# UCL-SML/Doubly-Stochastic-DGP

Hardware: AMD Instinct MI355X
Metric: ELBO-steps/sec (higher is better)
Workload: dtype f64

## Files before the change

doubly-stochastic-dgp_amd/csrc/model_kernels.hpp:

```cpp
#pragma once
__device__ __forceinline__ double softplus_d(double x) { return x > 0 ? x + log1p(exp(-x)) : log1p(exp(x)); }
__device__ __forceinline__ double sigmoid_d(double x) { return 1.0 / (1.0 + exp(-x)); }
__device__ __forceinline__ double kvar_of(const LayerDev& v, const double* __restrict__ theta) {
  const double rv = theta[v.off_kvar];
  return v.kvar_identity ? rv : softplus_d(rv) + SOFTPLUS_LOWER;
}

template <bool WAVE_TILES>
__device__ void prep_body(const LayerDev& v, const double* __restrict__ theta, double* __restrict__ lik_const, int64_t off_lik,
                          int lik_gauss, int bx, int nprep) {
  const int tid0 = bx * blockDim.x + threadIdx.x, nth = nprep * blockDim.x;
  if (tid0 == 0) {
    const double rv = theta[v.off_kvar];
    const double var = kvar_of(v, theta);
    double wv = 0.0, dwv = 0.0;
    if (v.has_white) {
      const double rw = theta[v.off_wvar];
      wv = softplus_d(rw) + SOFTPLUS_LOWER;
      dwv = sigmoid_d(rw);
    }
    v.hyp[HYP_VAR] = var; v.hyp[HYP_WVAR] = wv; v.hyp[HYP_KDIAG] = var + wv;
    v.hyp[HYP_DVAR] = v.kvar_identity ? 1.0 : sigmoid_d(rv); v.hyp[HYP_DWVAR] = dwv;
    if (blockIdx.y == 0 && lik_gauss) {
      const double rl = theta[off_lik];
// ... 968 lines not shown
      }
      s = sum_wave(s);
      if (lane == 0) gl_s[q] = -2.0 * ils[q] * ils[q] * ils[q] * s + v.hyp_red[2 + q];
    }
    __syncthreads();
    if (threadIdx.x < Din) {
      const double gl = gl_s[threadIdx.x];
      if (v.ard)
        grad[v.off_kls + threadIdx.x] = gl * v.hyp[HYP_ILS + Din + threadIdx.x];
      else
        iso = gl;
    }
  } else {
    for (int q = threadIdx.x; q < Din; q += 256) {
      double s = 0.0;
      for (int b0 = 0; b0 < parts; b0 += 8) {
        double x[8];
#pragma unroll
        for (int u = 0; u < 8; ++u) x[u] = v.hyp2part[(b0 + u < parts ? b0 + u : parts - 1) * stride + 2 + q];
#pragma unroll
        for (int u = 0; u < 8; ++u)
          if (b0 + u < parts) s += x[u];
      }
      const double gl = -2.0 * ils[q] * ils[q] * ils[q] * s + v.hyp_red[2 + q];
      if (v.ard)
        grad[v.off_kls + q] = gl * v.hyp[HYP_ILS + Din + q];
      else
        iso += gl;
    }
  }
  iso = block_sum_256(iso, sh);
  if (!v.ard && threadIdx.x == 0) grad[v.off_kls] = iso * v.hyp[HYP_ILS + Din];
}
__device__ __forceinline__ void adam_sweep(double* __restrict__ theta, const double* __restrict__ grad, double* __restrict__ m,
                                           double* __restrict__ v, const double* __restrict__ mask, int64_t n, double lr_t, double b1,
                                           double b2, double eps, double want, int64_t first, int64_t nthreads) {
  typedef double d2 __attribute__((ext_vector_type(2)));
  const int64_t npair = n >> 1;
  for (int64_t k0 = first; k0 < npair; k0 += 4 * nthreads) {
    d2 mk[4];
    bool act[4];
#pragma unroll
    for (int u = 0; u < 4; ++u) {
      const int64_t k = k0 + u * nthreads;
      mk[u] = *reinterpret_cast<const d2*>(mask + 2 * (k < npair ? k : first));
    }
#pragma unroll
    for (int u = 0; u < 4; ++u) {
      const int64_t k = k0 + u * nthreads;
      act[u] = k < npair && (want == 0.0 ? (mk[u][0] != 0.0 || mk[u][1] != 0.0) : (mk[u][0] == want || mk[u][1] == want));
    }
    d2 g[4], mm[4], vv[4], th[4];
#pragma unroll
    for (int u = 0; u < 4; ++u) {
      const int64_t k = k0 + u * nthreads;
      if (act[u]) {
        g[u] = *reinterpret_cast<const d2*>(grad + 2 * k);
        mm[u] = *reinterpret_cast<const d2*>(m + 2 * k);
        vv[u] = *reinterpret_cast<const d2*>(v + 2 * k);
        th[u] = *reinterpret_cast<const d2*>(theta + 2 * k);
      }
    }
#pragma unroll
    for (int u = 0; u < 4; ++u) {
      if (!act[u]) continue;
      const int64_t k = k0 + u * nthreads;
      bool on[2];
#pragma unroll
      for (int e = 0; e < 2; ++e) {
        on[e] = want == 0.0 ? mk[u][e] != 0.0 : mk[u][e] == want;
        if (on[e]) {
          const double mi = b1 * mm[u][e] + (1.0 - b1) * g[u][e];
          const double vi = b2 * vv[u][e] + (1.0 - b2) * g[u][e] * g[u][e];
          mm[u][e] = mi;
          vv[u][e] = vi;
          th[u][e] -= lr_t * mi / (sqrt(vi) + eps);
        }
      }
      if (on[0] && on[1]) {
        *reinterpret_cast<d2*>(m + 2 * k) = mm[u];
        *reinterpret_cast<d2*>(v + 2 * k) = vv[u];
        *reinterpret_cast<d2*>(theta + 2 * k) = th[u];
      } else {
#pragma unroll
        for (int e = 0; e < 2; ++e)
          if (on[e]) {
            m[2 * k + e] = mm[u][e];
            v[2 * k + e] = vv[u][e];
            theta[2 * k + e] = th[u][e];
          }
      }
    }
  }
  if ((n & 1) && first == 0) {
    const int64_t i = n - 1;
    const bool on = want == 0.0 ? mask[i] != 0.0 : mask[i] == want;
    if (on) {
      const double gi = grad[i];
      const double mi = b1 * m[i] + (1.0 - b1) * gi;
      const double vi = b2 * v[i] + (1.0 - b2) * gi * gi;
      m[i] = mi;
      v[i] = vi;
      theta[i] -= lr_t * mi / (sqrt(vi) + eps);
    }
  }
}
__device__ __forceinline__ bool chol_failed(const LayerDev* __restrict__ layers, int L) {
  bool bad = false;
  for (int l = 0; l < L; ++l) bad |= layers[l].scal[1] != 0.0;
  return bad;
}
__global__ void k_adam(double* __restrict__ theta, const double* __restrict__ grad, double* __restrict__ m,
                       double* __restrict__ v, const double* __restrict__ mask, int64_t n, double lr_t, double b1,
                       double b2, double eps, const LayerDev* __restrict__ layers, int L) {
  if (chol_failed(layers, L)) return;
  adam_sweep(theta, grad, m, v, mask, n, lr_t, b1, b2, eps, 0.0, (int64_t)blockIdx.x * blockDim.x + threadIdx.x,
             (int64_t)gridDim.x * blockDim.x);
}

__global__ __launch_bounds__(256) void k_asm_rows(const LayerDev* __restrict__ layers, double* __restrict__ grad, double kl_w, int mp_max, int pre_on) {
  extern __shared__ __attribute__((aligned(16))) double asm_dyn[];
  __shared__ double sh[4];
  const LayerDev v = layers[blockIdx.y];
  const int tid = threadIdx.x, lane = tid & 63, wave = tid >> 6;
  const int i = (int)blockIdx.x;
  const int Mp = v.Mp, M = v.M, Din = v.D_in, Dout = v.D_out;
  if (i >= M) return;
  lptr wm = (lptr)asm_dyn;
  const int64_t MM = (int64_t)Mp * Mp;
  const double kvar = v.hyp[HYP_VAR];
  const bool pre = pre_on && (M <= 128) && (Din <= 8) && (Dout * M <= 1024);
  double pz[2][2] = {{0, 0}, {0, 0}}, pzi[2] = {0, 0}, ptz[2] = {0, 0}, ptz1 = 0.0, pq_t = 0.0, pq_n = 0.0;
  double p4p[4] = {0, 0, 0, 0}, p4u[4] = {0, 0, 0, 0}, p4t[4] = {0, 0, 0, 0};
  if (pre) {
    gcptr Zp = (gcptr)v.Zp, thinz = (gcptr)v.thinz, thinq = (gcptr)v.thinq, n4 = (gcptr)v.n4, PT = (gcptr)v.PT, U = (gcptr)v.U, Tp = (gcptr)v.Tp;
#pragma unroll
    for (int u = 0; u < 2; ++u) {
      const int q = wave + 4 * u, qc = q < Din ? q : Din - 1;
      pzi[u] = Zp[i * Din + qc];
      ptz[u] = thinz[i * v.DinP16 + qc];
#pragma unroll
      for (int w = 0; w < 2; ++w) {
        const int j = lane + 64 * w;
        pz[u][w] = Zp[(j < M ? j : M - 1) * Din + qc];
      }
    }
    ptz1 = thinz[i * v.DinP16 + Din];
    const int dq = tid < Dout ? tid : Dout - 1;
    pq_t = thinq[i * v.DP16 + dq];
    pq_n = n4[i * v.DP4 + dq];
#pragma unroll
    for (int u = 0; u < 4; ++u) {
      int e = tid + 256 * u;
      e = e < Dout * M ? e : Dout * M - 1;
      const int d = e / M, j = e - d * M;
      const int64_t p = d * MM + (int64_t)i * Mp + (j <= i ? j : i);
      p4p[u] = PT[p];
      p4u[u] = U[p];
      p4t[u] = Tp[p];
    }
  }
  double a_sum = 0.0, tr = 0.0;
  for (int j = tid; j < M; j += 256) {
    const int64_t idx = (int64_t)i * Mp + j, idt = (int64_t)j * Mp + i;
    double nn = 0.0, uu = 0.0, gsym;
    if (v.alg_g) {
      double gs = 0.0, nt = 0.0;
#pragma unroll 4
      for (int d = 0; d < Dout; ++d) {
        const double ni = v.n4[i * v.DP4 + d], nj = v.n4[j * v.DP4 + d];
        const double g1 = v.GS[d * MM + idx], g2 = v.GS[d * MM + idt], pd = v.bigred[MM + d * MM + idx];
        const double tj = v.thinq[j * v.DP16 + d], ti2 = v.thinq[i * v.DP16 + d];
        nn = fma(ni, nj, nn);
        uu += v.UU[d * MM + idx];
        gs += (g1 + g2) - pd;
        nt += ni * tj + nj * ti2;
      }
      gsym = gs + 0.5 * nt;
    } else {
#pragma unroll 4
      for (int d = 0; d < Dout; ++d) {
        nn = fma(v.n4[i * v.DP4 + d], v.n4[j * v.DP4 + d], nn);
        uu += v.UU[d * MM + idx];
      }
      gsym = 0.5 * (v.bigred[idx] + v.bigred[idt]);
    }
    const double kb = -gsym + kl_w * (0.5 * Dout * v.Kinv[idx] - 0.5 * uu - 0.5 * nn);
    double k, dk;
    if (v.kern_kind == DSDGP_KERN_RBF)
      kern_val_grad<DSDGP_KERN_RBF>(v.R2[idx], kvar, k, dk);
    else
      kern_val_grad<DSDGP_KERN_MATERN52>(v.R2[idx], kvar, k, dk);
    wm[j] = kb * dk;
    a_sum += kb * k / kvar;
    if (j == i) tr = kb;
  }
  a_sum = block_sum_256(a_sum, sh);
  tr = block_sum_256(tr, sh);
  double* __restrict__ hp = v.hyp2part + (int64_t)i * (Din + 2);
  if (tid == 0) {
    hp[0] = a_sum;
    hp[1] = tr;
  }
  const double* __restrict__ ils = v.hyp + HYP_ILS;
  if (pre) {
#pragma unroll
    for (int u = 0; u < 2; ++u) {
      const int q = wave + 4 * u;
      if (q >= Din) break;
      const double zi = pzi[u];
      double s1 = 0.0, s2 = 0.0;
#pragma unroll
      for (int w = 0; w < 2; ++w) {
        const int j = lane + 64 * w;
        if (j < M) {
          const double df = zi - pz[u][w], wj = wm[j];
          s1 = fma(wj, df, s1);
          s2 = fma(wj * df, df, s2);
        }
      }
      s1 = sum_wave(s1);
      s2 = sum_wave(s2);
      if (lane == 0) {
        const double il2 = ils[q] * ils[q];
        grad[v.off_Z + (int64_t)i * Din + q] = 4.0 * il2 * s1 - 2.0 * il2 * (ptz[u] - zi * ptz1);
        hp[2 + q] = s2;
      }
    }
    if (tid < Dout) grad[v.off_q_mu + (int64_t)i * Dout + tid] = pq_t + kl_w * pq_n;
#pragma unroll
    for (int u = 0; u < 4; ++u) {
      const int e = tid + 256 * u;
      if (e < Dout * M) {
        const int d = e / M, j = e - d * M;
        const double gq = 2.0 * p4p[u] + kl_w * (p4u[u] - (i == j ? 1.0 / p4t[u] : 0.0));
        grad[v.off_q_sqrt + ((int64_t)d * M + i) * M + j] = (j <= i) ? gq : 0.0;
      }
    }
  } else {
  for (int q = wave; q < Din; q += 4) {
    const double zi = v.Zp[i * Din + q];
    double s1 = 0.0, s2 = 0.0;
    for (int j = lane; j < M; j += 64) {
      const double df = zi - v.Zp[j * Din + q], w = wm[j];
      s1 = fma(w, df, s1);
      s2 = fma(w * df, df, s2);
    }
    s1 = sum_wave(s1);
    s2 = sum_wave(s2);
    if (lane == 0) {
      const double il2 = ils[q] * ils[q];
      grad[v.off_Z + (int64_t)i * Din + q] = 4.0 * il2 * s1 - 2.0 * il2 * (v.thinz[i * v.DinP16 + q] - zi * v.thinz[i * v.DinP16 + Din]);
      hp[2 + q] = s2;
    }
  }
  for (int d = tid; d < Dout; d += 256) grad[v.off_q_mu + (int64_t)i * Dout + d] = v.thinq[i * v.DP16 + d] + kl_w * v.n4[i * v.DP4 + d];
  {
    constexpr int NU = 4;
    for (int j0 = 0; j0 < M; j0 += 256 * NU) {
      double pt[NU], uu[NU], td = 0.0;
      auto request = [&](int d) {
        gcptr PT = (gcptr)(v.PT + d * MM + (int64_t)i * Mp), U = (gcptr)(v.U + d * MM + (int64_t)i * Mp);
#pragma unroll
        for (int u = 0; u < NU; ++u) {
          const int j = j0 + tid + 256 * u, jc = j <= i ? j : i;
          pt[u] = PT[jc];
          uu[u] = U[jc];
        }
        td = ((gcptr)v.Tp)[d * MM + (int64_t)i * Mp + i];
      };
      request(0);
      for (int d = 0; d < Dout; ++d) {
        double gq[NU];
        const double tinv = 1.0 / td;
#pragma unroll
        for (int u = 0; u < NU; ++u) {
          const int j = j0 + tid + 256 * u;
          gq[u] = (j <= i) ? 2.0 * pt[u] + kl_w * (uu[u] - (i == j ? tinv : 0.0)) : 0.0;
        }
        if (d + 1 < Dout) request(d + 1);
        double* gr = grad + v.off_q_sqrt + ((int64_t)d * M + i) * M;
#pragma unroll
        for (int u = 0; u < NU; ++u) {
          const int j = j0 + tid + 256 * u;
          if (j < M) gr[j] = gq[u];
        }
      }
    }
  }
  }
  if (v.meanAB) {
    if (v.off_mean_A >= 0)
      for (int64_t idx = (int64_t)i * 256 + tid; idx < (int64_t)Din * Dout; idx += (int64_t)M * 256)
        grad[v.off_mean_A + idx] = v.meanAB[(idx / Dout) * v.DP16 + idx % Dout];
    if (v.off_mean_b >= 0 && i == 0)
      for (int idx = tid; idx < Dout; idx += 256) grad[v.off_mean_b + idx] = v.meanAB[(int64_t)Din * v.DP16 + idx];
  }
}

struct AdamArgs {
  double* theta; double* m; double* v; const double* mask;
  int64_t n;
  double lr_t, b1, b2, eps;
  int32_t on;
};
__device__ __forceinline__ void adam_one(const AdamArgs& A, int64_t i, double g) {
  const double mi = A.b1 * A.m[i] + (1.0 - A.b1) * g;
  const double vi = A.b2 * A.v[i] + (1.0 - A.b2) * g * g;
  A.m[i] = mi;
  A.v[i] = vi;
  A.theta[i] -= A.lr_t * mi / (sqrt(vi) + A.eps);
}
struct FinArgs {
  const double* part; int nblocks; double w, kl_weight; const double* lik_const; int64_t off_lik; double* out; int L;
  int do_fin;
};
__global__ __launch_bounds__(256) void k_tail(const LayerDev* __restrict__ layers_all, int first, int La, double* __restrict__ grad,
                                              const FinArgs F, const AdamArgs A) {
  __shared__ double sh[4];
  const int b = (int)blockIdx.x;
  const bool adam_on = A.on && !chol_failed(layers_all, F.L);
  if (b < La) {
    const LayerDev v = layers_all[first + b];
    asm_hyp_final(v, grad);
    if (adam_on) {
      __syncthreads();
      const int Din = v.D_in;
      if (threadIdx.x == 0) {
        if (A.mask[v.off_kvar] != 0.0) adam_one(A, v.off_kvar, grad[v.off_kvar]);
        if (v.has_white && A.mask[v.off_wvar] != 0.0) adam_one(A, v.off_wvar, grad[v.off_wvar]);
        if (!v.ard && A.mask[v.off_kls] != 0.0) adam_one(A, v.off_kls, grad[v.off_kls]);
      }
      if (v.ard && (int)threadIdx.x < Din && A.mask[v.off_kls + threadIdx.x] != 0.0)
        adam_one(A, v.off_kls + threadIdx.x, grad[v.off_kls + threadIdx.x]);
    }
    return;
  }
  const int nf = F.do_fin ? 1 : 0;
  if (b == La && nf) {
    double a = 0.0, c = 0.0;
    for (int i = threadIdx.x; i < F.nblocks; i += 256) {
      a += F.part[2 * i];
      c += F.part[2 * i + 1];
    }
    a = block_sum_256(a, sh);
    c = block_sum_256(c, sh);
    const double kl = layers_kl_value(layers_all, F.L, sh);
    if (threadIdx.x == 0) {
      double info = 0.0;
      for (int l = 0; l < F.L; ++l)
        if (layers_all[l].scal[1] != 0.0 && info == 0.0) info = layers_all[l].scal[1];
      F.out[0] = F.w * a - F.kl_weight * kl;
      F.out[1] = F.w * a;
      F.out[2] = F.kl_weight * kl;
      F.out[3] = info;
      if (F.off_lik >= 0) {
        const double g = -F.w * c * F.lik_const[1];
        grad[F.off_lik] = g;
        if (adam_on && A.mask[F.off_lik] != 0.0) adam_one(A, F.off_lik, g);
      }
    }
    return;
  }
  if (!adam_on) return;
  adam_sweep(A.theta, grad, A.m, A.v, A.mask, A.n, A.lr_t, A.b1, A.b2, A.eps, 1.0, (int64_t)(b - La - nf) * 256 + threadIdx.x,
             (int64_t)(gridDim.x - La - nf) * 256);
}
```

doubly-stochastic-dgp_amd/csrc/model_layout.hpp:

```cpp
#pragma once
static void layout(dsdgp_model* m, char* base, size_t* total) {
  Bump b{base, 0};
  const dsdgp_model_desc& D = m->desc;
  m->layers_dev = b.take<LayerDev>(D.L);
  m->mask = b.take<double>(D.n_theta);
  m->lik_const = b.take<double>(8);
  m->scal4 = b.take<double>(8);
  const int64_t Rlast = (int64_t)m->s_max * m->n_max;
  m->lik_blocks_max = std::max(ceil_div((Rlast + 16) * D.layers[D.L - 1].D_out, 256) + 1,
                               4 * ceil_div(Rlast, 16) + 4);
  m->lik_part = b.take<double>((size_t)m->lik_blocks_max * 2);
  m->Xmb = b.take<double>((size_t)m->n_max * D.layers[0].D_in);
  m->Ymb = b.take<double>((size_t)m->n_max * D.layers[D.L - 1].D_out);
  m->lik_dmean = b.take<double>((size_t)Rlast * D.layers[D.L - 1].D_out);
  m->lik_dvar = b.take<double>((size_t)Rlast * D.layers[D.L - 1].D_out);
  m->potrf_items = b.take<PotrfItem>(D.L);
  m->gp_fwd = b.take<GemmProblem>(4 * D.L);
  m->gp_bwd1 = b.take<GemmProblem>(4 * D.L);
  m->gp_pt = b.take<GemmProblem>(2 * D.L);
  m->gp_bwd2 = b.take<GemmProblem>(D.L);
  m->gp_wz = b.take<GemmProblem>(D.L);
  m->gp_w1 = b.take<GemmProblem>(2 * D.L); m->gp_w2 = b.take<GemmProblem>(D.L); m->gp_w3 = b.take<GemmProblem>(D.L);
  m->rjobs_cap = 0;
  for (int l = 0; l < D.L; ++l) m->rjobs_cap += D.layers[l].D_out + 5;
  m->rjobs = b.take<RedJob>(m->rjobs_cap);
  bool uniform = D.L > 1 && pad_M(D.layers[0].M) >= big_mp(true);
  for (int l = 1; l < D.L; ++l) uniform = uniform && D.layers[l].M == D.layers[0].M;
  uniform = uniform && pad_M(D.layers[0].M) % 64 == 0;
  m->uniform_big = uniform;
  double *Kp_all = nullptr, *Linv_all = nullptr, *LinvT_all = nullptr, *scal_all = nullptr;
  if (uniform) {
    const size_t MM0 = (size_t)pad_M(D.layers[0].M) * pad_M(D.layers[0].M);
    Kp_all = b.take<double>(D.L * MM0); Linv_all = b.take<double>(D.L * MM0); LinvT_all = b.take<double>(D.L * MM0);
    scal_all = b.take<double>(D.L * 8);
  }
  for (int l = 0; l < D.L; ++l) {
    LayerState& S = m->L[l];
    const dsdgp_layer_desc& d = D.layers[l];
    S.d = d;
    LayerDev& v = S.dev;
// ... 122 lines not shown
```

doubly-stochastic-dgp_amd/csrc/model_schedule.hpp:

```cpp
#pragma once
static bool overlap_on(const dsdgp_model* m, int64_t n, int S) {
  const char* no = getenv("DSDGP_NO_OVERLAP");
  if (!m->overlap || (no && atoi(no))) return false;
  int mp_max = 0;
  for (int l = 0; l < m->desc.L; ++l) mp_max = std::max(mp_max, (int)m->L[l].dev.Mp);
  return n * S * (int64_t)mp_max >= (int64_t)m->force.overlap_min;
}

static int join_prep(dsdgp_model* m) {
  if (m->side_pending) {
    DS_HIP(hipStreamWaitEvent(m->ctx->stream, m->ev_prep_side, 0));
    m->side_pending = false;
  }
  return DSDGP_OK;
}

static int prepare_async(dsdgp_model* m, bool with_grad = false, bool side = false, const HeadRand* hr = nullptr,
                         const HeadGather* hg = nullptr) {
  dsdgp_ctx* ctx = m->ctx;
  const int L = m->desc.L;
  DS_TRY(join_prep(m));
  const bool keep_kuu = m->track_theta && m->kuu_valid;
  const bool unchanged = keep_kuu && m->q_dirty == -1 && (m->prepared_grad || !with_grad);
  int mp_max = 0;
// ... 399 lines not shown
  return DSDGP_OK;
}

static int launch_finalize(dsdgp_model* m, hipStream_t st) {
  DS_LAUNCH(k_finalize, dim3(1), dim3(256), 0, st, m->layers_dev, m->desc.L, m->lik_part, m->fin.nblocks, m->fin.w,
                     m->fin.kl_weight, m->lik_const, m->grad,
                     lik_has_param(m->desc.lik_kind) ? m->desc.off_lik_var : (int64_t)-1, m->fin.with_grad, m->fin.out);
  DS_HIP(hipGetLastError());
  m->fin.done = true;
  return DSDGP_OK;
}

static int backward_layers(dsdgp_model* m, int64_t n, int S, double kl_weight) {
  dsdgp_ctx* ctx = m->ctx;
  const int L = m->desc.L;
  DS_TRY(ensure_plan(m, n, S));
  const bool overlap = overlap_on(m, n, S);
  const int gfirst0 = m->desc.white ? 0 : m->grad_first;
  const bool tail_in_loop = (m->bucket_fn != nullptr && m->tail_ok && gfirst0 == 0 && !m->fuse_adam.on) ||
                            (overlap && m->force.pipe_tail != 0 && !m->desc.white);
  const bool kinv_only = overlap && !tail_in_loop && !m->desc.white && m->kinv_pending && m->side_pending;
  if (kinv_only) DS_HIP(hipStreamWaitEvent(ctx->stream, m->ev_kinv, 0));
  else DS_TRY(join_prep(m));
  const int gfirst = m->desc.white ? 0 : m->grad_first;
  const bool bucketed = m->bucket_fn != nullptr && m->tail_ok && gfirst == 0 && !m->fuse_adam.on;
  const bool pipelined = bucketed || (overlap && m->force.pipe_tail != 0 && !m->desc.white);
  auto layer_tail = [&](LayerState& St, hipStream_t st) -> int {
    DS_LAUNCH(k_reduce_grouped, dim3(St.red_blkn), dim3(256), m->red_lds, st, m->rjobs + St.red_off, St.red_n, St.red_blk0);
    DS_HIP(hipGetLastError());
    DS_TRY(gemm_launch(ctx, St.lq + St.lq_nf + St.lq_n1 + St.lq_n2, St.lq_np, St.lq_tp, st));
    if (bucketed) {
      const int l = (int)(&St - m->L);
      const LayerDev* lay1 = m->layers_dev + l;
      DS_LAUNCH(k_asm_rows, dim3(St.dev.M, 1), dim3(256), (size_t)m->mp_max_all * sizeof(double), st, lay1, m->grad, kl_weight,
                         m->mp_max_all, m->force.asm_pre);
      FinArgs F{};
      AdamArgs A{};
      DS_LAUNCH(k_tail, dim3(1), dim3(256), 0, st, m->layers_dev, l, 1, m->grad, F, A);
      DS_HIP(hipGetLastError());
      const int64_t lo = St.d.off_Z;
      const int64_t hi = (l + 1 < L) ? m->L[l + 1].d.off_Z
                                     : (lik_has_param(m->desc.lik_kind) ? m->desc.off_lik_var : m->desc.n_theta);
      m->bucket_fn(m->bucket_user, l, m->grad + lo, hi - lo, (void*)st);
    }
    return DSDGP_OK;
  };
  const bool q_only = m->grad_q_only && !m->desc.white;
  auto launch_wgrad = [&](LayerState& Sx, hipStream_t st) -> int {
    const int64_t ldx = Sx.ld_used;
    if (q_only && &Sx == &m->L[gfirst]) return wgrad_launch(ctx, Sx.wj, Sx.njobsA, Sx.totA, Sx.ns_big, ldx, ldx, st);
    return wgrad_launch(ctx, Sx.wj, Sx.njobs, Sx.tot_big, Sx.ns_big, ldx, ldx, st);
  };
  const bool defer_upper = overlap && !pipelined && (m->force.wg_defer == 2 || (m->force.wg_defer < 0 && L - gfirst >= 4));
  for (int l = L - 1; l >= gfirst; --l) {
    LayerState& St = m->L[l];
    const LayerDev& v = St.dev;
    const bool last = (l == L - 1);
    const int64_t Rin = St.Rin_used, ld = St.ld_used;
    const int rep = St.rep_used;
    const bool fused = (last && m->fused_last) || (!last && l >= 1);
    const bool skip_chain = q_only && l == gfirst;
    const bool in_chain = !fused && !last && !skip_chain && m->force.adj_fuse != 0 && !St.c_used && !St.gemm &&
                          sm_adj_fusable(v.Mp, ld / 16, v.D_in, v.D_out);
    if (!fused && !in_chain)
      DS_LAUNCH(k_adj_prep, dim3(ceil_div(ld, 256), std::max(v.DP16, v.DinP16)), dim3(256), 0, ctx->stream, last ? nullptr : St.dF,
                         last ? m->lik_dmean : nullptr, last ? m->lik_dvar : nullptr, St.z_used, St.zs_s, St.zs_n,
                         St.zs_d, n, St.var, St.X_used, Rin, rep, v.D_in, v.D_out, v.DP16, v.DinP16, m->desc.jitter, ld,
                         St.MB, St.VB, St.XT1, v.D_out + St.prop, St.prop);
    DS_HIP(hipGetLastError());
    const bool on_main = overlap && l == gfirst && L - gfirst > 1;
// ... 68 lines not shown
    }
    DS_HIP(hipGetLastError());
    if (m->desc.white) {
      DS_LAUNCH(k_white_lbar, dim3(32, L), dim3(256), 0, ctx->stream, m->layers_dev);
      DS_TRY(gemm_launch(ctx, m->gp_w1, 2 * L, m->t_w1));
      DS_LAUNCH(k_white_phi, dim3(32, L), dim3(256), 0, ctx->stream, m->layers_dev);
      DS_TRY(gemm_launch(ctx, m->gp_w2, L, m->t_w2));
      DS_TRY(gemm_launch(ctx, m->gp_w3, L, m->t_w3));
    } else if (gfirst > 0) {
      for (int l = gfirst; l < L; ++l) {
        LayerState& Sq = m->L[l];
        DS_TRY(gemm_launch(ctx, Sq.lq + Sq.lq_nf + Sq.lq_n1 + Sq.lq_n2, Sq.lq_np, Sq.lq_tp));
      }
    } else {
      DS_TRY(gemm_launch(ctx, m->gp_pt, m->n_pt, m->t_pt));
    }
  }
  const LayerDev* lay = m->layers_dev + gfirst;
  const int La = L - gfirst;
  if (bucketed) {
    FinArgs F{m->lik_part, m->fin.nblocks, m->fin.w, m->fin.kl_weight, m->lik_const,
              lik_has_param(m->desc.lik_kind) ? m->desc.off_lik_var : (int64_t)-1, m->fin.out, L, 1};
    AdamArgs A{};
    DS_LAUNCH(k_tail, dim3(1), dim3(256), 0, ctx->stream, m->layers_dev, 0, 0, m->grad, F, A);
    DS_HIP(hipGetLastError());
    m->fin.done = true;
    const int64_t lo = lik_has_param(m->desc.lik_kind) ? m->desc.off_lik_var : m->desc.n_theta;
    const bool tail_scalars = m->fin.out == m->grad + m->desc.n_theta;
    m->bucket_fn(m->bucket_user, L, m->grad + lo, (m->desc.n_theta - lo) + (tail_scalars ? 4 : 0), (void*)ctx->stream);
    if (!tail_scalars) m->bucket_fn(m->bucket_user, L + 1, m->fin.out, 4, (void*)ctx->stream);
    return DSDGP_OK;
  }
  if (m->tail_ok) {
    DS_LAUNCH(k_asm_rows, dim3(m->m_max_all, La), dim3(256), (size_t)m->mp_max_all * sizeof(double), ctx->stream, lay, m->grad,
                       kl_weight, m->mp_max_all, m->force.asm_pre);
    FinArgs F{m->lik_part, m->fin.nblocks, m->fin.w, m->fin.kl_weight, m->lik_const,
              lik_has_param(m->desc.lik_kind) ? m->desc.off_lik_var : (int64_t)-1, m->fin.out, L, 1};
    AdamArgs A{m->theta, m->adam_m, m->adam_v, m->mask, m->desc.n_theta, m->fuse_adam.lr_t, m->fuse_adam.b1, m->fuse_adam.b2,
               m->fuse_adam.eps, (m->fuse_adam.on && gfirst == 0) ? 1 : 0};
    const int nadam = A.on ? (int)std::min<int64_t>(2048, ceil_div(m->desc.n_theta, 512)) : 0;
    DS_LAUNCH(k_tail, dim3(La + 1 + nadam), dim3(256), 0, ctx->stream, m->layers_dev, gfirst, La, m->grad, F, A);
    DS_HIP(hipGetLastError());
    m->fin.done = true;
    return DSDGP_OK;
  }
  DS_LAUNCH(k_asm_kbar, dim3(m->kuu_blocks, La), dim3(256), 0, ctx->stream, lay, kl_weight);
  if (m->n_wz) DS_TRY(gemm_launch(ctx, m->gp_wz, m->n_wz, m->t_wz));
  if (m->need_hyp_part) DS_LAUNCH(k_asm_hyp_part, dim3(NPART, La), dim3(256), 0, ctx->stream, lay);
  DS_LAUNCH(k_asm_params, dim3(m->asm_blocks + 1, La), dim3(256), 0, ctx->stream, lay, m->grad, kl_weight);
  DS_HIP(hipGetLastError());
  return DSDGP_OK;
}

struct GatherSrc {
  const double *Xs, *Ys;
  const int64_t* idx;
};
static int elbo_impl(dsdgp_model* m, const double* X, const double* Y, int64_t n, int32_t S, const double* const* zs,
                     const int64_t* zstride, uint64_t seed, double data_scale, double kl_weight, int with_grad, double* out,
                     const GatherSrc* gs) {
  DS_CHECK_ARG(m && out && ((X && Y) || gs));
  DS_CHECK_ARG(!zs || zstride);
  DS_CHECK_ARG(!m->sample_w || S == m->sample_w_S);
  if (with_grad) {
    DS_CHECK_ARG(m->grad != nullptr);
  }
  dsdgp_ctx* ctx = m->ctx;
  const int L = m->desc.L;
  bool z_side = false, z_head = false;
  const bool ovl = overlap_on(m, n, S);
  HeadRand hr{};
  if (m->head_ok) {
// ... 146 lines not shown
```

doubly-stochastic-dgp_amd/csrc/model_types.hpp:

```cpp
#pragma once
struct LayerDev {
  int32_t M, Mp, D_in, D_out, DP4, DP16, DinP16, kern_kind, ard, has_white, white, hyp_parts;
  int32_t kl_parts, kvar_identity;
  int64_t off_Z, off_q_mu, off_q_sqrt, off_kvar, off_kls, off_wvar;
  double *Zp, *Zs, *hyp, *Tp, *TpT, *qmu, *qmu4;
  double *Kp, *Linv, *LinvT, *Kinv, *scal;
  double *V, *nL, *Sd, *klv;
  double *U, *n4, *PT, *UU, *Kbar, *wm, *wk;
  double *bigred, *thinq, *thinz, *hyp_red;
  double* meanAB;
  int64_t off_mean_A, off_mean_b;
  double *R2, *Zp1, *WZ;
  double *klpart, *hyp2part;
  double *KS, *GS;
  int32_t alg_g, need_tpt;
  double *wLbar, *wH, *wY, *wX;
  double *ngTI, *ngTinv, *ngTbar, *ngH, *ngY, *ngX, *ngSinv, *ngA, *ngLAinv, *ngLAinvT, *ngV , *ngTheta1 , *ngScal ;
};
#define NPART 32
#define PREP_BLOCKS 64
#define WIDE_DIN 32

struct RedJob {
  const double* part;
// ... 61 lines not shown
  double* lik_part;
  int lik_blocks_max;
  double *lik_dmean, *lik_dvar;
  double* scal4;
  PotrfItem* potrf_items;
  GemmProblem *gp_fwd, *gp_bwd1, *gp_bwd2, *gp_w1, *gp_w2, *gp_w3;
  GemmProblem* gp_pt;
  int n_pt = 0, t_pt = 0;
  hipEvent_t ev_fork, ev_prep_side, ev_z;
  hipEvent_t ev_kinv;
  bool kinv_pending = false;
  int32_t* gemm_order = nullptr;
  int64_t gemm_order_cap = 0, gemm_order_used = 0;
  GemmLayerWs gws{};
  bool prepared_grad = false;
  bool track_theta = false;
  bool kuu_valid = false;
  int grad_first = 0;
  bool grad_pruned = false;
  bool grad_q_only = false;
  int q_dirty = -2;
  bool side_pending = false;
  int n_fwd, n_bwd1, n_bwd2, t_fwd, t_bwd1, t_bwd2, n_w, t_w1, t_w2, t_w3;
  const double* sample_w = nullptr;
  int sample_w_S = 0;
  GemmProblem* gp_wz;
  int n_wz = 0, t_wz = 0, kuu_blocks = 32, asm_blocks = 64, prep_blocks = PREP_BLOCKS;
  bool uniform_big = false;
  BigChol big_all;
  bool need_hyp_part = false;
  bool tail_ok = false;
  struct { int on; double lr_t, b1, b2, eps; } fuse_adam = {0, 0, 0, 0, 0};
  int mp_max_all = 0, m_max_all = 0;
  dsdgp_bucket_fn bucket_fn = nullptr;
  void* bucket_user = nullptr;
  double *Xmb = nullptr, *Ymb = nullptr;
  bool head_ok = false;
  bool last_deferred = false;
  LayerFwdArgs last_fwd;
  bool fused_last = false;
  struct { int nblocks; double w, kl_weight; int with_grad; double* out; bool done; } fin;
  RedJob* rjobs;
  int rjobs_cap, n_red, red_blocks;
  size_t red_lds = 0;
  int64_t plan_n;
  int plan_S;
  bool prepared;
  hipStream_t side;
  hipEvent_t ev_bwd[DSDGP_MAX_LAYERS];
  hipEvent_t ev_side;
  bool overlap;
  struct Force { int save_c = 1, cs_min_blocks = 160, cs_min_dout = 3, cs_max_dout = 1 << 20, wg_defer = -1, alg_g = -1, bwd_split = 1, pipe_tail = 0, head = 1, tail = 1, adj_fuse = 1, ext_ev = 1, lik_fuse = 1, red_ahead = 1, white_fwd = 1, gemm_mp = 512, last_fuse = 1, last_min_blocks = 1, asm_pre = 1, overlap_min = 1 << 18, wg_red = 1, wg_group = 1; } force;
};
static void parse_force(dsdgp_model* m) {
  const char* e = getenv("DSDGP_FORCE");
  if (!e) return;
  std::string str(e);
  size_t pos = 0;
  while (pos < str.size()) {
    size_t end = str.find(',', pos);
    if (end == std::string::npos) end = str.size();
    const std::string kv = str.substr(pos, end - pos);
    const size_t eq = kv.find('=');
    if (eq != std::string::npos) {
      const std::string k = kv.substr(0, eq);
      const int v = atoi(kv.c_str() + eq + 1);
      if (k == "save_c") m->force.save_c = v;
      else if (k == "cs_min_blocks") m->force.cs_min_blocks = v;
      else if (k == "cs_min_dout") m->force.cs_min_dout = v;
      else if (k == "cs_max_dout") m->force.cs_max_dout = v;
      else if (k == "wg_defer") m->force.wg_defer = v;
      else if (k == "alg_g") m->force.alg_g = v;
      else if (k == "bwd_split") m->force.bwd_split = v;
      else if (k == "red_ahead") m->force.red_ahead = v;
      else if (k == "white_fwd") m->force.white_fwd = v;
      else if (k == "pipe_tail") m->force.pipe_tail = v;
      else if (k == "head") m->force.head = v;
      else if (k == "tail") m->force.tail = v;
      else if (k == "adj_fuse") m->force.adj_fuse = v;
      else if (k == "ext_ev") m->force.ext_ev = v;
      else if (k == "lik_fuse") m->force.lik_fuse = v;
      else if (k == "gemm_mp") m->force.gemm_mp = v;
      else if (k == "last_fuse") m->force.last_fuse = v;
      else if (k == "last_min_blocks") m->force.last_min_blocks = v;
      else if (k == "asm_pre") m->force.asm_pre = v;
      else if (k == "overlap_min") m->force.overlap_min = v;
      else if (k == "wg_red") m->force.wg_red = v;
      else if (k == "wg_group") m->force.wg_group = v;
    }
    pos = end + 1;
  }
}

struct Bump {
  char* base;
  size_t off;
  template <class T>
  T* take(size_t count) {
    off = (size_t)round_up((int64_t)off, 256);
    T* p = base ? (T*)(base + off) : nullptr;
    off += count * sizeof(T);
    return p;
  }
};

static bool save_c_enabled(const dsdgp_model* m, int Mp) {
  return m->force.save_c >= 2 || (m->force.save_c == 1 && Mp > 256);
}
static int chain_d_split(int64_t nblk, int D_out) {
  int ds = 1;
  if (nblk < 256) ds = (int)std::min<int64_t>(4, std::max<int64_t>(1, 512 / nblk));
  else if (nblk < 512) ds = (int)std::min<int64_t>(1024 / nblk, D_out / 5);
  if (ds > D_out) ds = D_out;
  return ds < 1 ? 1 : ds;
}
static inline bool lik_has_param(int kind) {
  return kind == DSDGP_LIK_GAUSSIAN || kind == DSDGP_LIK_STUDENT_T || kind == DSDGP_LIK_GAMMA || kind == DSDGP_LIK_BETA;
}
static inline bool lik_is_generic(int kind) { return kind >= DSDGP_LIK_POISSON && kind <= DSDGP_LIK_BETA; }
static int big_mp(bool uniform) {
  static const int nonuniform = getenv("DSDGP_BIG_MP") ? atoi(getenv("DSDGP_BIG_MP")) : 192;
// ... 15 lines not shown
```

Baseline: 2031.

## Fuse hyperparameter tail, ELBO finalize and Adam into row-assembly kernel

The row-assembly kernel now applies the Adam update to each Z, q_mu, q_sqrt and mean parameter right after writing its gradient. Adam state for the pre-loaded path is fetched ahead of the gradient math. A per-layer atomic counter picks the last finishing row block, which then runs the hyperparameter gradient finalization and its Adam step. An extra grid column computes the ELBO value and the likelihood-variance gradient. Together these remove the separate tail kernel launch and its full-parameter Adam sweep, at the cost of atomics, extra register pressure and cross-block ordering that depends on fences.

```diff
diff --git a/doubly-stochastic-dgp_amd/csrc/model_kernels.hpp b/doubly-stochastic-dgp_amd/csrc/model_kernels.hpp
--- a/doubly-stochastic-dgp_amd/csrc/model_kernels.hpp
+++ b/doubly-stochastic-dgp_amd/csrc/model_kernels.hpp
@@ -1024,6 +1024,36 @@
   iso = block_sum_256(iso, sh);
   if (!v.ard && threadIdx.x == 0) grad[v.off_kls] = iso * v.hyp[HYP_ILS + Din];
 }
+__device__ __forceinline__ void adam_update(double g, double& m, double& v, double& th, double lr_t, double b1, double b2, double eps) {
+  const double mi = b1 * m + (1.0 - b1) * g;
+  const double vi = b2 * v + (1.0 - b2) * g * g;
+  m = mi;
+  v = vi;
+  th -= lr_t * mi / (sqrt(vi) + eps);
+}
+struct AdamArgs {
+  double* theta; double* m; double* v; const double* mask;
+  int64_t n;
+  double lr_t, b1, b2, eps;
+  int32_t on;
+};
+__device__ __forceinline__ void adam_one(const AdamArgs& A, int64_t i, double g) {
+  double mi = A.m[i], vi = A.v[i], th = A.theta[i];
+  adam_update(g, mi, vi, th, A.lr_t, A.b1, A.b2, A.eps);
+  A.m[i] = mi;
+  A.v[i] = vi;
+  A.theta[i] = th;
+}
+__device__ __forceinline__ void adam_put(const AdamArgs& A, int64_t i, double g, double mi, double vi, double th) {
+  adam_update(g, mi, vi, th, A.lr_t, A.b1, A.b2, A.eps);
+  A.m[i] = mi;
+  A.v[i] = vi;
+  A.theta[i] = th;
+}
+struct FinArgs {
+  const double* part; int nblocks; double w, kl_weight; const double* lik_const; int64_t off_lik; double* out; int L;
+  int do_fin;
+};
 __device__ __forceinline__ void adam_sweep(double* __restrict__ theta, const double* __restrict__ grad, double* __restrict__ m,
                                            double* __restrict__ v, const double* __restrict__ mask, int64_t n, double lr_t, double b1,
                                            double b2, double eps, double want, int64_t first, int64_t nthreads) {
@@ -1062,11 +1092,11 @@
       for (int e = 0; e < 2; ++e) {
         on[e] = want == 0.0 ? mk[u][e] != 0.0 : mk[u][e] == want;
         if (on[e]) {
-          const double mi = b1 * mm[u][e] + (1.0 - b1) * g[u][e];
-          const double vi = b2 * vv[u][e] + (1.0 - b2) * g[u][e] * g[u][e];
+          double mi = mm[u][e], vi = vv[u][e], ti = th[u][e];
+          adam_update(g[u][e], mi, vi, ti, lr_t, b1, b2, eps);
           mm[u][e] = mi;
           vv[u][e] = vi;
-          th[u][e] -= lr_t * mi / (sqrt(vi) + eps);
+          th[u][e] = ti;
         }
       }
       if (on[0] && on[1]) {
@@ -1088,12 +1118,11 @@
     const int64_t i = n - 1;
     const bool on = want == 0.0 ? mask[i] != 0.0 : mask[i] == want;
     if (on) {
-      const double gi = grad[i];
-      const double mi = b1 * m[i] + (1.0 - b1) * gi;
-      const double vi = b2 * v[i] + (1.0 - b2) * gi * gi;
+      double mi = m[i], vi = v[i], ti = theta[i];
+      adam_update(grad[i], mi, vi, ti, lr_t, b1, b2, eps);
       m[i] = mi;
       v[i] = vi;
-      theta[i] -= lr_t * mi / (sqrt(vi) + eps);
+      theta[i] = ti;
     }
   }
 }
@@ -1109,15 +1138,63 @@
   adam_sweep(theta, grad, m, v, mask, n, lr_t, b1, b2, eps, 0.0, (int64_t)blockIdx.x * blockDim.x + threadIdx.x,
              (int64_t)gridDim.x * blockDim.x);
 }
-
-__global__ __launch_bounds__(256) void k_asm_rows(const LayerDev* __restrict__ layers, double* __restrict__ grad, double kl_w, int mp_max, int pre_on) {
+__device__ __forceinline__ void tail_hyp(const LayerDev& v, double* __restrict__ grad, const AdamArgs& A, bool adam_on) {
+  asm_hyp_final(v, grad);
+  if (!adam_on) return;
+  __syncthreads();
+  const int Din = v.D_in;
+  if (threadIdx.x == 0) {
+    if (A.mask[v.off_kvar] != 0.0) adam_one(A, v.off_kvar, grad[v.off_kvar]);
+    if (v.has_white && A.mask[v.off_wvar] != 0.0) adam_one(A, v.off_wvar, grad[v.off_wvar]);
+    if (!v.ard && A.mask[v.off_kls] != 0.0) adam_one(A, v.off_kls, grad[v.off_kls]);
+  }
+  if (v.ard && (int)threadIdx.x < Din && A.mask[v.off_kls + threadIdx.x] != 0.0)
+    adam_one(A, v.off_kls + threadIdx.x, grad[v.off_kls + threadIdx.x]);
+}
+__device__ __forceinline__ void tail_value(const LayerDev* __restrict__ layers_all, double* __restrict__ grad, const FinArgs& F,
+                                           const AdamArgs& A, bool adam_on, double* sh) {
+  double a = 0.0, c = 0.0;
+  for (int i = threadIdx.x; i < F.nblocks; i += 256) {
+    a += F.part[2 * i];
+    c += F.part[2 * i + 1];
+  }
+  a = block_sum_256(a, sh);
+  c = block_sum_256(c, sh);
+  const double kl = layers_kl_value(layers_all, F.L, sh);
+  if (threadIdx.x == 0) {
+    double info = 0.0;
+    for (int l = 0; l < F.L; ++l)
+      if (layers_all[l].scal[1] != 0.0 && info == 0.0) info = layers_all[l].scal[1];
+    F.out[0] = F.w * a - F.kl_weight * kl;
+    F.out[1] = F.w * a;
+    F.out[2] = F.kl_weight * kl;
+    F.out[3] = info;
+    if (F.off_lik >= 0) {
+      const double g = -F.w * c * F.lik_const[1];
+      grad[F.off_lik] = g;
+      if (adam_on && A.mask[F.off_lik] != 0.0) adam_one(A, F.off_lik, g);
+    }
+  }
+}
+
+__global__ __launch_bounds__(256) void k_asm_rows(const LayerDev* __restrict__ layers, double* __restrict__ grad, double kl_w, int mp_max, int pre_on,
+                                                  const LayerDev* __restrict__ layers_all, int32_t* __restrict__ cnt, int fin_rows,
+                                                  const FinArgs F, const AdamArgs A) {
   extern __shared__ __attribute__((aligned(16))) double asm_dyn[];
   __shared__ double sh[4];
+  __shared__ int s_last;
+  const bool adam_on = fin_rows && A.on && !chol_failed(layers_all, F.L);
+  if (fin_rows && blockIdx.x == gridDim.x - 1) {
+    if (blockIdx.y == 0) tail_value(layers_all, grad, F, A, adam_on, sh);
+    return;
+  }
   const LayerDev v = layers[blockIdx.y];
   const int tid = threadIdx.x, lane = tid & 63, wave = tid >> 6;
   const int i = (int)blockIdx.x;
   const int Mp = v.Mp, M = v.M, Din = v.D_in, Dout = v.D_out;
   if (i >= M) return;
+  const bool ad_z = adam_on && A.mask[v.off_Z] != 0.0, ad_qm = adam_on && A.mask[v.off_q_mu] != 0.0,
+             ad_qs = adam_on && A.mask[v.off_q_sqrt] != 0.0;
   lptr wm = (lptr)asm_dyn;
   const int64_t MM = (int64_t)Mp * Mp;
   const double kvar = v.hyp[HYP_VAR];
@@ -1150,6 +1227,33 @@
       p4p[u] = PT[p];
       p4u[u] = U[p];
       p4t[u] = Tp[p];
+    }
+  }
+  double zm[2] = {0, 0}, zv[2] = {0, 0}, zt[2] = {0, 0}, qm_m = 0.0, qm_v = 0.0, qm_t = 0.0;
+  double sm[4] = {0, 0, 0, 0}, sv[4] = {0, 0, 0, 0}, st[4] = {0, 0, 0, 0};
+  if (pre && adam_on) {
+    gcptr Am = (gcptr)A.m, Av = (gcptr)A.v, At = (gcptr)A.theta;
+    if (ad_z) {
+#pragma unroll
+      for (int u = 0; u < 2; ++u) {
+        const int q = wave + 4 * u;
+        const int64_t e = v.off_Z + (int64_t)i * Din + (q < Din ? q : Din - 1);
+        zm[u] = Am[e]; zv[u] = Av[e]; zt[u] = At[e];
+      }
+    }
+    if (ad_qm) {
+      const int64_t e = v.off_q_mu + (int64_t)i * Dout + (tid < Dout ? tid : Dout - 1);
+      qm_m = Am[e]; qm_v = Av[e]; qm_t = At[e];
+    }
+    if (ad_qs) {
+#pragma unroll
+      for (int u = 0; u < 4; ++u) {
+        int e = tid + 256 * u;
+        e = e < Dout * M ? e : Dout * M - 1;
+        const int d = e / M, j = e - d * M;
+        const int64_t p = v.off_q_sqrt + ((int64_t)d * M + i) * M + (j <= i ? j : i);
+        sm[u] = Am[p]; sv[u] = Av[p]; st[u] = At[p];
+      }
     }
   }
   double a_sum = 0.0, tr = 0.0;
@@ -1190,9 +1294,13 @@
   a_sum = block_sum_256(a_sum, sh);
   tr = block_sum_256(tr, sh);
   double* __restrict__ hp = v.hyp2part + (int64_t)i * (Din + 2);
+  auto hp_put = [&](int k, double x) {
+    if (fin_rows) __hip_atomic_store(hp + k, x, __ATOMIC_RELAXED, __HIP_MEMORY_SCOPE_AGENT);
+    else hp[k] = x;
+  };
   if (tid == 0) {
-    hp[0] = a_sum;
-    hp[1] = tr;
+    hp_put(0, a_sum);
+    hp_put(1, tr);
   }
   const double* __restrict__ ils = v.hyp + HYP_ILS;
   if (pre) {
@@ -1215,23 +1323,38 @@
       s2 = sum_wave(s2);
       if (lane == 0) {
         const double il2 = ils[q] * ils[q];
-        grad[v.off_Z + (int64_t)i * Din + q] = 4.0 * il2 * s1 - 2.0 * il2 * (ptz[u] - zi * ptz1);
-        hp[2 + q] = s2;
-      }
-    }
-    if (tid < Dout) grad[v.off_q_mu + (int64_t)i * Dout + tid] = pq_t + kl_w * pq_n;
+        const double gz = 4.0 * il2 * s1 - 2.0 * il2 * (ptz[u] - zi * ptz1);
+        const int64_t e = v.off_Z + (int64_t)i * Din + q;
+        grad[e] = gz;
+        hp_put(2 + q, s2);
+        if (ad_z) adam_put(A, e, gz, zm[u], zv[u], zt[u]);
+      }
+    }
+    if (tid < Dout) {
+      const double gm = pq_t + kl_w * pq_n;
+      const int64_t e = v.off_q_mu + (int64_t)i * Dout + tid;
+      grad[e] = gm;
+      if (ad_qm) adam_put(A, e, gm, qm_m, qm_v, qm_t);
+    }
 #pragma unroll
     for (int u = 0; u < 4; ++u) {
       const int e = tid + 256 * u;
       if (e < Dout * M) {
         const int d = e / M, j = e - d * M;
         const double gq = 2.0 * p4p[u] + kl_w * (p4u[u] - (i == j ? 1.0 / p4t[u] : 0.0));
-        grad[v.off_q_sqrt + ((int64_t)d * M + i) * M + j] = (j <= i) ? gq : 0.0;
+        const int64_t p = v.off_q_sqrt + ((int64_t)d * M + i) * M + j;
+        grad[p] = (j <= i) ? gq : 0.0;
+        if (ad_qs && j <= i) adam_put(A, p, gq, sm[u], sv[u], st[u]);
       }
     }
   } else {
   for (int q = wave; q < Din; q += 4) {
     const double zi = v.Zp[i * Din + q];
+    const int64_t ez = v.off_Z + (int64_t)i * Din + q;
+    double am = 0.0, av = 0.0, at = 0.0;
+    if (ad_z && lane == 0) {
+      am = A.m[ez]; av = A.v[ez]; at = A.theta[ez];
+    }
     double s1 = 0.0, s2 = 0.0;
     for (int j = lane; j < M; j += 64) {
       const double df = zi - v.Zp[j * Din + q], w = wm[j];
@@ -1242,15 +1365,25 @@
     s2 = sum_wave(s2);
     if (lane == 0) {
       const double il2 = ils[q] * ils[q];
-      grad[v.off_Z + (int64_t)i * Din + q] = 4.0 * il2 * s1 - 2.0 * il2 * (v.thinz[i * v.DinP16 + q] - zi * v.thinz[i * v.DinP16 + Din]);
-      hp[2 + q] = s2;
-    }
-  }
-  for (int d = tid; d < Dout; d += 256) grad[v.off_q_mu + (int64_t)i * Dout + d] = v.thinq[i * v.DP16 + d] + kl_w * v.n4[i * v.DP4 + d];
+      const double gz = 4.0 * il2 * s1 - 2.0 * il2 * (v.thinz[i * v.DinP16 + q] - zi * v.thinz[i * v.DinP16 + Din]);
+      grad[ez] = gz;
+      hp_put(2 + q, s2);
+      if (ad_z) adam_put(A, ez, gz, am, av, at);
+    }
+  }
+  for (int d = tid; d < Dout; d += 256) {
+    const double gm = v.thinq[i * v.DP16 + d] + kl_w * v.n4[i * v.DP4 + d];
+    const int64_t e = v.off_q_mu + (int64_t)i * Dout + d;
+    grad[e] = gm;
+    if (ad_qm) adam_one(A, e, gm);
+  }
   {
     constexpr int NU = 4;
     for (int j0 = 0; j0 < M; j0 += 256 * NU) {
       double pt[NU], uu[NU], td = 0.0;
+      double am[NU], av[NU], at[NU];
+#pragma unroll
+      for (int u = 0; u < NU; ++u) am[u] = av[u] = at[u] = 0.0;
       auto request = [&](int d) {
         gcptr PT = (gcptr)(v.PT + d * MM + (int64_t)i * Mp), U = (gcptr)(v.U + d * MM + (int64_t)i * Mp);
 #pragma unroll
@@ -1260,6 +1393,16 @@
           uu[u] = U[jc];
         }
         td = ((gcptr)v.Tp)[d * MM + (int64_t)i * Mp + i];
+        if (ad_qs) {
+          const int64_t r = v.off_q_sqrt + ((int64_t)d * M + i) * M;
+#pragma unroll
+          for (int u = 0; u < NU; ++u) {
+            const int j = j0 + tid + 256 * u;
+            if (j <= i) {
+              am[u] = ((gcptr)A.m)[r + j]; av[u] = ((gcptr)A.v)[r + j]; at[u] = ((gcptr)A.theta)[r + j];
+            }
+          }
+        }
       };
       request(0);
       for (int d = 0; d < Dout; ++d) {
@@ -1269,13 +1412,25 @@
         for (int u = 0; u < NU; ++u) {
           const int j = j0 + tid + 256 * u;
           gq[u] = (j <= i) ? 2.0 * pt[u] + kl_w * (uu[u] - (i == j ? tinv : 0.0)) : 0.0;
+          if (ad_qs && j <= i) adam_update(gq[u], am[u], av[u], at[u], A.lr_t, A.b1, A.b2, A.eps);
+        }
+        double nm[NU], nv[NU], nt[NU];
+#pragma unroll
+        for (int u = 0; u < NU; ++u) {
+          nm[u] = am[u]; nv[u] = av[u]; nt[u] = at[u];
         }
         if (d + 1 < Dout) request(d + 1);
-        double* gr = grad + v.off_q_sqrt + ((int64_t)d * M + i) * M;
+        const int64_t r = v.off_q_sqrt + ((int64_t)d * M + i) * M;
+        double* gr = grad + r;
 #pragma unroll
         for (int u = 0; u < NU; ++u) {
           const int j = j0 + tid + 256 * u;
           if (j < M) gr[j] = gq[u];
+          if (ad_qs && j <= i) {
+            A.m[r + j] = nm[u];
+            A.v[r + j] = nv[u];
+            A.theta[r + j] = nt[u];
+          }
         }
       }
     }
@@ -1283,30 +1438,36 @@
   }
   if (v.meanAB) {
     if (v.off_mean_A >= 0)
-      for (int64_t idx = (int64_t)i * 256 + tid; idx < (int64_t)Din * Dout; idx += (int64_t)M * 256)
-        grad[v.off_mean_A + idx] = v.meanAB[(idx / Dout) * v.DP16 + idx % Dout];
+      for (int64_t idx = (int64_t)i * 256 + tid; idx < (int64_t)Din * Dout; idx += (int64_t)M * 256) {
+        const double g = v.meanAB[(idx / Dout) * v.DP16 + idx % Dout];
+        grad[v.off_mean_A + idx] = g;
+        if (adam_on && A.mask[v.off_mean_A + idx] != 0.0) adam_one(A, v.off_mean_A + idx, g);
+      }
     if (v.off_mean_b >= 0 && i == 0)
-      for (int idx = tid; idx < Dout; idx += 256) grad[v.off_mean_b + idx] = v.meanAB[(int64_t)Din * v.DP16 + idx];
-  }
-}
-
-struct AdamArgs {
-  double* theta; double* m; double* v; const double* mask;
-  int64_t n;
-  double lr_t, b1, b2, eps;
-  int32_t on;
-};
-__device__ __forceinline__ void adam_one(const AdamArgs& A, int64_t i, double g) {
-  const double mi = A.b1 * A.m[i] + (1.0 - A.b1) * g;
-  const double vi = A.b2 * A.v[i] + (1.0 - A.b2) * g * g;
-  A.m[i] = mi;
-  A.v[i] = vi;
-  A.theta[i] -= A.lr_t * mi / (sqrt(vi) + A.eps);
-}
-struct FinArgs {
-  const double* part; int nblocks; double w, kl_weight; const double* lik_const; int64_t off_lik; double* out; int L;
-  int do_fin;
-};
+      for (int idx = tid; idx < Dout; idx += 256) {
+        const double g = v.meanAB[(int64_t)Din * v.DP16 + idx];
+        grad[v.off_mean_b + idx] = g;
+        if (adam_on && A.mask[v.off_mean_b + idx] != 0.0) adam_one(A, v.off_mean_b + idx, g);
+      }
+  }
+  if (!fin_rows) return;
+  asm volatile("s_waitcnt vmcnt(0)" ::: "memory");
+  __syncthreads();
+  if (tid == 0) {
+    const int t = __hip_atomic_fetch_add(cnt + blockIdx.y, 1, __ATOMIC_RELAXED, __HIP_MEMORY_SCOPE_AGENT);
+    const int last = t == M - 1;
+    if (last) {
+      __builtin_amdgcn_fence(__ATOMIC_ACQUIRE, "agent");
+      asm volatile("s_waitcnt vmcnt(0)" ::: "memory");
+      __hip_atomic_store(cnt + blockIdx.y, 0, __ATOMIC_RELAXED, __HIP_MEMORY_SCOPE_AGENT);
+    }
+    s_last = last;
+  }
+  __syncthreads();
+  if (!s_last) return;
+  tail_hyp(v, grad, A, adam_on);
+}
+
 __global__ __launch_bounds__(256) void k_tail(const LayerDev* __restrict__ layers_all, int first, int La, double* __restrict__ grad,
                                               const FinArgs F, const AdamArgs A) {
   __shared__ double sh[4];
@@ -1314,44 +1475,12 @@
   const bool adam_on = A.on && !chol_failed(layers_all, F.L);
   if (b < La) {
     const LayerDev v = layers_all[first + b];
-    asm_hyp_final(v, grad);
-    if (adam_on) {
-      __syncthreads();
-      const int Din = v.D_in;
-      if (threadIdx.x == 0) {
-        if (A.mask[v.off_kvar] != 0.0) adam_one(A, v.off_kvar, grad[v.off_kvar]);
-        if (v.has_white && A.mask[v.off_wvar] != 0.0) adam_one(A, v.off_wvar, grad[v.off_wvar]);
-        if (!v.ard && A.mask[v.off_kls] != 0.0) adam_one(A, v.off_kls, grad[v.off_kls]);
-      }
-      if (v.ard && (int)threadIdx.x < Din && A.mask[v.off_kls + threadIdx.x] != 0.0)
-        adam_one(A, v.off_kls + threadIdx.x, grad[v.off_kls + threadIdx.x]);
-    }
+    tail_hyp(v, grad, A, adam_on);
     return;
   }
   const int nf = F.do_fin ? 1 : 0;
   if (b == La && nf) {
-    double a = 0.0, c = 0.0;
-    for (int i = threadIdx.x; i < F.nblocks; i += 256) {
-      a += F.part[2 * i];
-      c += F.part[2 * i + 1];
-    }
-    a = block_sum_256(a, sh);
-    c = block_sum_256(c, sh);
-    const double kl = layers_kl_value(layers_all, F.L, sh);
-    if (threadIdx.x == 0) {
-      double info = 0.0;
-      for (int l = 0; l < F.L; ++l)
-        if (layers_all[l].scal[1] != 0.0 && info == 0.0) info = layers_all[l].scal[1];
-      F.out[0] = F.w * a - F.kl_weight * kl;
-      F.out[1] = F.w * a;
-      F.out[2] = F.kl_weight * kl;
-      F.out[3] = info;
-      if (F.off_lik >= 0) {
-        const double g = -F.w * c * F.lik_const[1];
-        grad[F.off_lik] = g;
-        if (adam_on && A.mask[F.off_lik] != 0.0) adam_one(A, F.off_lik, g);
-      }
-    }
+    tail_value(layers_all, grad, F, A, adam_on, sh);
     return;
   }
   if (!adam_on) return;
diff --git a/doubly-stochastic-dgp_amd/csrc/model_layout.hpp b/doubly-stochastic-dgp_amd/csrc/model_layout.hpp
--- a/doubly-stochastic-dgp_amd/csrc/model_layout.hpp
+++ b/doubly-stochastic-dgp_amd/csrc/model_layout.hpp
@@ -6,6 +6,7 @@
   m->mask = b.take<double>(D.n_theta);
   m->lik_const = b.take<double>(8);
   m->scal4 = b.take<double>(8);
+  m->tail_cnt = b.take<int32_t>(DSDGP_MAX_LAYERS);
   const int64_t Rlast = (int64_t)m->s_max * m->n_max;
   m->lik_blocks_max = std::max(ceil_div((Rlast + 16) * D.layers[D.L - 1].D_out, 256) + 1,
                                4 * ceil_div(Rlast, 16) + 4);
diff --git a/doubly-stochastic-dgp_amd/csrc/model_schedule.hpp b/doubly-stochastic-dgp_amd/csrc/model_schedule.hpp
--- a/doubly-stochastic-dgp_amd/csrc/model_schedule.hpp
+++ b/doubly-stochastic-dgp_amd/csrc/model_schedule.hpp
@@ -455,10 +455,10 @@
     if (bucketed) {
       const int l = (int)(&St - m->L);
       const LayerDev* lay1 = m->layers_dev + l;
-      DS_LAUNCH(k_asm_rows, dim3(St.dev.M, 1), dim3(256), (size_t)m->mp_max_all * sizeof(double), st, lay1, m->grad, kl_weight,
-                         m->mp_max_all, m->force.asm_pre);
       FinArgs F{};
       AdamArgs A{};
+      DS_LAUNCH(k_asm_rows, dim3(St.dev.M, 1), dim3(256), (size_t)m->mp_max_all * sizeof(double), st, lay1, m->grad, kl_weight,
+                         m->mp_max_all, m->force.asm_pre, (const LayerDev*)m->layers_dev, m->tail_cnt, 0, F, A);
       DS_LAUNCH(k_tail, dim3(1), dim3(256), 0, st, m->layers_dev, l, 1, m->grad, F, A);
       DS_HIP(hipGetLastError());
       const int64_t lo = St.d.off_Z;
@@ -593,12 +593,19 @@
     return DSDGP_OK;
   }
   if (m->tail_ok) {
-    DS_LAUNCH(k_asm_rows, dim3(m->m_max_all, La), dim3(256), (size_t)m->mp_max_all * sizeof(double), ctx->stream, lay, m->grad,
-                       kl_weight, m->mp_max_all, m->force.asm_pre);
     FinArgs F{m->lik_part, m->fin.nblocks, m->fin.w, m->fin.kl_weight, m->lik_const,
               lik_has_param(m->desc.lik_kind) ? m->desc.off_lik_var : (int64_t)-1, m->fin.out, L, 1};
     AdamArgs A{m->theta, m->adam_m, m->adam_v, m->mask, m->desc.n_theta, m->fuse_adam.lr_t, m->fuse_adam.b1, m->fuse_adam.b2,
                m->fuse_adam.eps, (m->fuse_adam.on && gfirst == 0) ? 1 : 0};
+    if (m->force.tail_rows != 0) {
+      DS_LAUNCH(k_asm_rows, dim3(m->m_max_all + 1, La), dim3(256), (size_t)m->mp_max_all * sizeof(double), ctx->stream, lay, m->grad,
+                         kl_weight, m->mp_max_all, m->force.asm_pre, (const LayerDev*)m->layers_dev, m->tail_cnt + gfirst, 1, F, A);
+      DS_HIP(hipGetLastError());
+      m->fin.done = true;
+      return DSDGP_OK;
+    }
+    DS_LAUNCH(k_asm_rows, dim3(m->m_max_all, La), dim3(256), (size_t)m->mp_max_all * sizeof(double), ctx->stream, lay, m->grad,
+                       kl_weight, m->mp_max_all, m->force.asm_pre, (const LayerDev*)m->layers_dev, m->tail_cnt, 0, F, A);
     const int nadam = A.on ? (int)std::min<int64_t>(2048, ceil_div(m->desc.n_theta, 512)) : 0;
     DS_LAUNCH(k_tail, dim3(La + 1 + nadam), dim3(256), 0, ctx->stream, m->layers_dev, gfirst, La, m->grad, F, A);
     DS_HIP(hipGetLastError());
diff --git a/doubly-stochastic-dgp_amd/csrc/model_types.hpp b/doubly-stochastic-dgp_amd/csrc/model_types.hpp
--- a/doubly-stochastic-dgp_amd/csrc/model_types.hpp
+++ b/doubly-stochastic-dgp_amd/csrc/model_types.hpp
@@ -117,6 +117,7 @@
   bool tail_ok = false;
   struct { int on; double lr_t, b1, b2, eps; } fuse_adam = {0, 0, 0, 0, 0};
   int mp_max_all = 0, m_max_all = 0;
+  int32_t* tail_cnt = nullptr;
   dsdgp_bucket_fn bucket_fn = nullptr;
   void* bucket_user = nullptr;
   double *Xmb = nullptr, *Ymb = nullptr;
@@ -135,7 +136,7 @@
   hipEvent_t ev_bwd[DSDGP_MAX_LAYERS];
   hipEvent_t ev_side;
   bool overlap;
-  struct Force { int save_c = 1, cs_min_blocks = 160, cs_min_dout = 3, cs_max_dout = 1 << 20, wg_defer = -1, alg_g = -1, bwd_split = 1, pipe_tail = 0, head = 1, tail = 1, adj_fuse = 1, ext_ev = 1, lik_fuse = 1, red_ahead = 1, white_fwd = 1, gemm_mp = 512, last_fuse = 1, last_min_blocks = 1, asm_pre = 1, overlap_min = 1 << 18, wg_red = 1, wg_group = 1; } force;
+  struct Force { int save_c = 1, cs_min_blocks = 160, cs_min_dout = 3, cs_max_dout = 1 << 20, wg_defer = -1, alg_g = -1, bwd_split = 1, pipe_tail = 0, head = 1, tail = 1, adj_fuse = 1, ext_ev = 1, lik_fuse = 1, red_ahead = 1, white_fwd = 1, gemm_mp = 512, last_fuse = 1, last_min_blocks = 1, asm_pre = 1, overlap_min = 1 << 18, wg_red = 1, wg_group = 1, tail_rows = 1; } force;
 };
 static void parse_force(dsdgp_model* m) {
   const char* e = getenv("DSDGP_FORCE");
@@ -172,6 +173,7 @@
       else if (k == "overlap_min") m->force.overlap_min = v;
       else if (k == "wg_red") m->force.wg_red = v;
       else if (k == "wg_group") m->force.wg_group = v;
+      else if (k == "tail_rows") m->force.tail_rows = v;
     }
     pos = end + 1;
   }
```

Result: no change. 2025 (-0.3%).
